# Brendonovich/spacedrive

Measured on AMD Instinct MI355X. Metric: cas_id files/sec + full-file BLAKE3 GB/s + dedup rows/sec at 1/2/4/8 MI355X, higher is better.
Workload: dtype u32; 1 GPU; identifier job step: config2 (1M files/GPU) cas_id + cas_id->Object grouping + Object write set (one fused pass on one GPU; at N > 1 hash-sharded over RCCL, each owner writing its share of the write set, padded exchange); parallelism=dp1 (files) + hash-sharded dedup, RCCL all-to-all

## Files before the change

### spacedrive_amd/csrc/b3_batch.hip

```cpp
#include <errno.h>
#include <stdlib.h>

#include <algorithm>
#include <atomic>

#include "b3_device.hpp"
#include "internal.hpp"
#include "scan_device.hpp"

namespace sdgpu {

namespace {

constexpr int kThreads = 256;

__device__ __forceinline__ void load_cv(const uint32_t* p, uint32_t cv[8]) {
  const uint4 a = reinterpret_cast<const uint4*>(p)[0];
  const uint4 b = reinterpret_cast<const uint4*>(p)[1];
  cv[0] = a.x; cv[1] = a.y; cv[2] = a.z; cv[3] = a.w;
  cv[4] = b.x; cv[5] = b.y; cv[6] = b.z; cv[7] = b.w;
}

__device__ __forceinline__ void store_cv(uint32_t* p, const uint32_t cv[8]) {
  reinterpret_cast<uint4*>(p)[0] = make_uint4(cv[0], cv[1], cv[2], cv[3]);
// ... 52 lines not shown
  if (rem == 0) return 0u;
  const uint32_t rem_bytes = len - 4 * q * B3_CHUNK_LEN;
  const uint32_t rem_blocks = rem_bytes == 0 ? 1u : (rem_bytes + 63) / 64;
  return rem_blocks + (rem - 1);
}

__device__ __forceinline__ void bins3(uint32_t len, bool ok, uint32_t& b0, uint32_t& b1) {
  b0 = b1 = kBins;
  if (!ok) return;
  const uint32_t lw = leaf_work3(len);
  if (lw) b0 = parent_bin(lw);
  const uint32_t q = units_of(len);
  if (q) b1 = parent_bin(q + (n_chunks_of(len) > 4 * q ? 1u : 0u));
}

struct Range3 {
  uint32_t lo, hi;
};
__device__ __forceinline__ Range3 block_range3(uint32_t n) {
  const uint32_t per = (n + gridDim.x - 1) / gridDim.x;
  const uint32_t lo = min(n, blockIdx.x * per);
  return {lo, min(n, lo + per)};
}

__device__ __forceinline__ bool msg_ok(uint64_t o, uint32_t l, uint32_t max_len,
                                       uint64_t arena_bytes) {
  return l <= max_len && (o & 15u) == 0 && o <= arena_bytes && l <= arena_bytes - o;
}

template <uint32_t kSkip>
constexpr uint32_t kAlignOf = kSkip ? 8u : 16u;

template <uint32_t kSkip>
__device__ __forceinline__ bool pass_msg(uint64_t o, uint32_t l, const uint8_t* __restrict__ whole,
                                         uint32_t i, uint32_t max_len, uint64_t arena_bytes,
                                         uint32_t& hl) {
  static_assert(kSkip == 0 || kSkip == 8, "the cas message or its body");
  bool ok = msg_ok(o, l, max_len, arena_bytes);
  hl = l;
  if constexpr (kSkip != 0) {
    ok = ok && l >= kSkip && whole[i] != 0;
    hl = l - kSkip;
  }
  return ok;
}

template <uint32_t kSkip>
__device__ __forceinline__ bool over_capacity(const uint32_t* d_units, uint32_t n, uint64_t cap,
                                              const uint32_t* grab) {
  if constexpr (kSkip != 0) return grab[1] != 0;
  return static_cast<uint64_t>(*d_units) + n > cap;
}

template <uint32_t kSkip>
__global__ __launch_bounds__(kThreads) void k_plan3(const uint64_t* __restrict__ off,
                                                    const uint32_t* __restrict__ len, uint32_t n,
                                                    uint32_t max_len, uint64_t arena_bytes,
                                                    uint32_t* __restrict__ units,
                                                    uint32_t* __restrict__ hist,
                                                    uint32_t* __restrict__ grab,
                                                    int32_t* __restrict__ status,
                                                    uint32_t out_words, uint32_t* __restrict__ out,
                                                    const uint8_t* __restrict__ whole,
                                                    uint8_t* __restrict__ has,
                                                    const uint32_t* d_units, uint64_t cap) {
  __shared__ uint32_t h[2][kBins];
  for (uint32_t t = threadIdx.x; t < 2 * kBins; t += kThreads) (&h[0][0])[t] = 0;
  if (blockIdx.x == 0 && threadIdx.x == 0) {
    *grab = 0;
    if constexpr (kSkip != 0) grab[1] = over_capacity<0>(d_units, n, cap, nullptr) ? 1u : 0u;
  }
  __syncthreads();
  const Range3 r = block_range3(n);
  for (uint32_t i = r.lo + threadIdx.x; i < r.hi; i += kThreads) {
    uint32_t l;
    const bool ok = pass_msg<kSkip>(off[i], len[i], whole, i, max_len, arena_bytes, l);
    units[i] = ok ? units_of(l) : 0u;
    if (status) status[i] = ok ? 0 : -EINVAL;
    if constexpr (kSkip != 0) has[i] = ok ? 1 : 0;
    if (!ok)
      for (uint32_t w = 0; w < out_words; ++w) out[i * out_words + w] = 0u;
    uint32_t b0, b1;
    bins3(l, ok, b0, b1);
    if (b0 < kBins) atomicAdd(&h[0][b0], 1u);
    if (b1 < kBins) atomicAdd(&h[1][b1], 1u);
  }
  __syncthreads();
  for (uint32_t t = threadIdx.x; t < 2 * kBins; t += kThreads)
    hist[static_cast<size_t>(t) * gridDim.x + blockIdx.x] = (&h[0][0])[t];
}

template <uint32_t kSkip>
__global__ __launch_bounds__(kThreads) void k_scatter3(const uint64_t* __restrict__ off,
                                                       const uint32_t* __restrict__ len, uint32_t n,
                                                       uint32_t max_len, uint64_t arena_bytes,
                                                       uint64_t cap, const uint32_t* __restrict__ d_units,
                                                       int32_t* __restrict__ status,
                                                       uint32_t out_words, uint32_t* __restrict__ out,
                                                       const uint32_t* __restrict__ unit_base,
                                                       const uint32_t* __restrict__ hist_scan,
                                                       uint32_t* __restrict__ order,
                                                       uint32_t* __restrict__ unit_msg,
                                                       const uint8_t* __restrict__ whole,
                                                       uint8_t* __restrict__ has,
                                                       const uint32_t* __restrict__ grab) {
  __shared__ uint32_t cur[2][kBins], cnt[2][kBins];
  const Range3 r = block_range3(n);
  if (over_capacity<kSkip>(d_units, n, cap, grab)) {
    for (uint32_t i = r.lo + threadIdx.x; i < r.hi; i += kThreads) {
      if (status) status[i] = -ENOBUFS;
      if constexpr (kSkip != 0) has[i] = 0;
      for (uint32_t w = 0; w < out_words; ++w) out[i * out_words + w] = 0u;
    }
    return;
  }
  for (uint32_t t = threadIdx.x; t < 2 * kBins; t += kThreads) {
    (&cur[0][0])[t] = hist_scan[static_cast<size_t>(t) * gridDim.x + blockIdx.x];
    (&cnt[0][0])[t] = 0;
  }
  __syncthreads();
  for (uint32_t i0 = r.lo; i0 < r.hi; i0 += kThreads) {
    const uint32_t i = i0 + threadIdx.x;
    uint32_t b0 = kBins, b1 = kBins, l0 = 0, l1 = 0;
    if (i < r.hi) {
      uint32_t l;
      const bool ok = pass_msg<kSkip>(off[i], len[i], whole, i, max_len, arena_bytes, l);
      bins3(l, ok, b0, b1);
      if (b0 < kBins) l0 = atomicAdd(&cnt[0][b0], 1u);
      if (b1 < kBins) l1 = atomicAdd(&cnt[1][b1], 1u);
      const uint32_t q = ok ? units_of(l) : 0u;
      const uint32_t ub = unit_base[i];
      for (uint32_t g = 0; g < q; ++g) unit_msg[ub + g] = i;
    }
    __syncthreads();
    if (b0 < kBins) order[cur[0][b0] + l0] = i;
    if (b1 < kBins) order[cur[1][b1] + l1] = i;
    __syncthreads();
    for (uint32_t t = threadIdx.x; t < 2 * kBins; t += kThreads) {
      (&cur[0][0])[t] += (&cnt[0][0])[t];
      (&cnt[0][0])[t] = 0;
    }
    __syncthreads();
  }
}

template <uint32_t kSkip>
__device__ __forceinline__ void unit_item(const uint8_t* __restrict__ arena,
                                          const uint64_t* __restrict__ off,
                                          const uint32_t* __restrict__ unit_msg,
                                          const uint32_t* __restrict__ unit_base, uint32_t u,
                                          uint32_t* __restrict__ cvs) {
  const uint32_t m = unit_msg[u];
  const uint32_t ub = unit_base[m];
  const uint32_t g = u - ub;
  const uint32_t j0 = 4 * g;
  const uint8_t* p = arena + off[m] + kSkip + static_cast<uint64_t>(j0) * B3_CHUNK_LEN;
  constexpr uint32_t kA = kAlignOf<kSkip>;
  uint32_t a[8], b[8], c[8];
  b3_chunk_full<kA>(p, j0, a);
  b3_chunk_full<kA>(p + 1024, j0 + 1, b);
  b3_parent(a, a, b, 0u);
  b3_chunk_full<kA>(p + 2048, j0 + 2, b);
  b3_chunk_full<kA>(p + 3072, j0 + 3, c);
  b3_parent(b, b, c, 0u);
  b3_parent(c, a, b, 0u);
  store_cv(cvs + static_cast<uint64_t>(ub + m + g) * 8, c);
}

template <uint32_t kAlign>
__device__ __forceinline__ void chunk_any(const uint8_t* __restrict__ p, uint32_t l, uint32_t j,
                                          uint32_t root_flag, uint32_t cv[8]) {
  const uint32_t clen = min(B3_CHUNK_LEN, l - j * B3_CHUNK_LEN);
  const uint8_t* cp = p + static_cast<uint64_t>(j) * B3_CHUNK_LEN;
  if (clen == B3_CHUNK_LEN && root_flag == 0)
    b3_chunk_full<kAlign>(cp, j, cv);
  else
    b3_chunk<kAlign>(cp, clen, j, root_flag, cv);
}

template <uint32_t kSkip>
__device__ __forceinline__ void msg_item(const uint8_t* __restrict__ arena,
                                         const uint64_t* __restrict__ off,
                                         const uint32_t* __restrict__ len,
                                         const uint32_t* __restrict__ unit_base, uint32_t m,
                                         uint32_t* __restrict__ cvs, uint32_t out_words,
                                         uint32_t* __restrict__ out) {
  const uint32_t l = len[m] - kSkip;
  const uint32_t nch = n_chunks_of(l), q = units_of(l);
  const uint32_t rem = nch - 4 * q;
  const uint8_t* p = arena + off[m] + kSkip;
  const uint32_t rootf = q == 0 ? B3_ROOT : 0u;
// ... 411 lines not shown
          break;
        }
        const uint64_t now = wall_clock64();
        if (now - t_last > idle_ticks || now - t_start > life_ticks) break;
        __builtin_amdgcn_s_sleep(2);
      }
      s_go = go;
    }
    __syncthreads();
    const uint32_t go = s_go;
    if (go == 0) break;
    const uint64_t t_seen = wall_clock64();
    const uint32_t l = min(s_len, kHostStageMax), out_words = min(s_words, 16u);
    stage_message(stage, msg, l);
    __syncthreads();
    const uint64_t t_loaded = wall_clock64();
    uint32_t h0 = 0, h1 = 0;
    quad_hash_staged(L, stage, l, cvr, h0, h1);
    if (t < 64) {
      uint32_t dg[8];
#pragma unroll
      for (int w = 0; w < 8; ++w) dg[w] = __shfl(w < 4 ? h0 : h1, w & 3);
      if (t == 0) {
        for (uint32_t w = 0; w < out_words; ++w)
          __hip_atomic_store(&mb->digest[w], w < 8 ? dg[w] : 0u, __ATOMIC_RELAXED,
                             __HIP_MEMORY_SCOPE_SYSTEM);
        __hip_atomic_store(&mb->t_seen, t_seen, __ATOMIC_RELAXED, __HIP_MEMORY_SCOPE_SYSTEM);
        __hip_atomic_store(&mb->t_loaded, t_loaded, __ATOMIC_RELAXED, __HIP_MEMORY_SCOPE_SYSTEM);
        __hip_atomic_store(&mb->t_done, wall_clock64(), __ATOMIC_RELAXED, __HIP_MEMORY_SCOPE_SYSTEM);
        __hip_atomic_store(&mb->done, go, __ATOMIC_RELEASE, __HIP_MEMORY_SCOPE_SYSTEM);
        last_seq = go;
      }
    }
    t_last = wall_clock64();
    __syncthreads();
  }
  if (t == 0) __hip_atomic_store(&mb->state, kSvcExited, __ATOMIC_RELEASE, __HIP_MEMORY_SCOPE_SYSTEM);
}

}

namespace {

template <uint32_t kSkip>
hipError_t batch_pass_launch(const uint8_t* arena, uint64_t arena_bytes, const uint64_t* off,
                             const uint32_t* len, const uint8_t* whole, uint32_t n,
                             uint32_t max_len, uint32_t out_words, uint8_t* out, uint8_t* has,
                             int32_t* status, const BatchWork& w, hipStream_t s, KTimer* timer) {
  if (n == 0) return hipSuccess;
  uint32_t* o = reinterpret_cast<uint32_t*>(out);
  const uint32_t nb = std::min<uint32_t>(kSortBlocks, (n + kThreads - 1) / kThreads);
  const uint32_t nh = 2 * kBins * nb;
  const uint64_t cap = w.max_chunks;
  k_plan3<kSkip><<<nb, kThreads, 0, s>>>(off, len, n, max_len, arena_bytes, w.n_chunks, w.hist,
                                         w.grab, status, out_words, o, whole, has, w.total, cap);
  scan::exclusive(w.n_chunks, n, w.chunk_base, w.block_sums, w.total, s);
  scan::exclusive(w.hist, nh, w.hist, w.hist_sums, nullptr, s);
  k_scatter3<kSkip><<<nb, kThreads, 0, s>>>(off, len, n, max_len, arena_bytes, cap, w.total, status,
                                            out_words, o, w.chunk_base, w.hist, w.order,
                                            w.chunk_msg, whole, has, w.grab);
  const uint32_t* d_r = w.hist + static_cast<size_t>(kBins) * nb;
  {
    KScope k(timer, kSkip ? "body_leaves" : "cas_leaves", s);
    k_leaves3<kSkip><<<leaves3_grid(), kThreads, 0, s>>>(arena, off, len, w.chunk_msg, w.chunk_base,
                                                         w.total, w.order, d_r, w.grab, w.cvs,
                                                         out_words, o, n, cap);
  }
  {
    KScope k(timer, kSkip ? "body_fold" : "cas_fold", s);
    k_fold3<kSkip><<<(n + kThreads - 1) / kThreads, kThreads, 0, s>>>(
        len, w.chunk_base, w.order, d_r, w.hist + nh, w.cvs, out_words, o, w.total, n, cap, w.grab);
  }
  return hipGetLastError();
}

}

hipError_t batch_hash_launch(const uint8_t* arena, uint64_t arena_bytes, const uint64_t* off,
                             const uint32_t* len, uint32_t n, uint32_t max_len,
                             uint32_t out_words, uint8_t* out, int32_t* status,
                             const BatchWork& w, hipStream_t s, KTimer* timer) {
  return batch_pass_launch<0>(arena, arena_bytes, off, len, nullptr, n, max_len, out_words, out,
                              nullptr, status, w, s, timer);
}

hipError_t batch_body_launch(const uint8_t* arena, uint64_t arena_bytes, const uint64_t* off,
                             const uint32_t* len, const uint8_t* whole, uint32_t n,
                             uint32_t max_len, uint8_t* out32, uint8_t* has, const BatchWork& w,
                             hipStream_t s, KTimer* timer) {
  return batch_pass_launch<8>(arena, arena_bytes, off, len, whole, n, max_len, 8, out32, has,
                              nullptr, w, s, timer);
}

}

namespace sdgpu {

size_t small_split_scratch_bytes() {
  return (kSplitMaxMsgs + static_cast<size_t>(kSplitMaxMsgs) * kSplitMaxGroups * 8) * 4;
}

hipError_t small_split_launch(const uint8_t* arena, const uint64_t* off, const uint32_t* len,
                              uint32_t n, uint32_t max_len, uint32_t max_chunks,
                              uint32_t out_words, uint8_t* out, int32_t* status, uint32_t* scratch,
                              hipStream_t s, KTimer* timer) {
  if (n == 0) return hipSuccess;
  if (n > kSplitMaxMsgs || max_chunks > kSmallMaxChunks || !scratch) return hipErrorInvalidValue;
  const uint32_t gmax = std::max<uint32_t>(1, (max_chunks + kSplitGroupChunks - 1) / kSplitGroupChunks);
  KScope k(timer, "cas_small_split", s);
  k_small_split<<<n * gmax, kSplitThreads, 0, s>>>(arena, off, len, max_len, gmax, out_words,
                                                   reinterpret_cast<uint32_t*>(out), status, scratch);
  return hipGetLastError();
}
// ... 51 lines not shown
```

### spacedrive_amd/csrc/bucket_part_device.hpp

```cpp
#pragma once

#include "part_device.hpp"

namespace sdgpu {
namespace {

constexpr uint32_t kMaxBucketBits = 15;

template <typename In, bool kInitRep>
__global__ __launch_bounds__(kPartThreads) void k_part_scatter_rec(
    In in, uint64_t n, uint32_t skip, uint32_t bits, const uint32_t* __restrict__ offs,
    uint4* __restrict__ rec, uint32_t* __restrict__ rep) {
  extern __shared__ __attribute__((aligned(16))) uint32_t cur[];
  const uint32_t nbins = 1u << bits;
  for (uint32_t b = threadIdx.x; b < nbins; b += kPartThreads)
    cur[b] = offs[static_cast<uint64_t>(b) * gridDim.x + part_block()];
  __syncthreads();
  uint64_t t0, t1;
  tile_of(n, gridDim.x, t0, t1);
  constexpr int U = kUnroll;
  for (uint64_t i0 = t0 + threadIdx.x; i0 < t1; i0 += U * kPartThreads) {
    RowBatch<U> q;
    in.template load_many<U>(i0, kPartThreads, t1, i0, q);
#pragma unroll
    for (int u = 0; u < U; ++u) {
      const uint64_t i = i0 + static_cast<uint64_t>(u) * kPartThreads;
      const uint32_t r = in.rank_of(q, u);
      if (kInitRep && q.in[u]) rep[i] = r;
      if (!in.valid_of(q, u)) continue;
      const uint64_t h = in_hash<In>(in.key_of(q, u));
      const uint32_t p = atomicAdd(&cur[digit_of(h, skip, bits)], 1u);
      rec[p] = make_uint4(static_cast<uint32_t>(h), static_cast<uint32_t>(h >> 32), r,
                          in.row_of(q, u));
    }
  }
}

constexpr uint32_t kRunMaxBins = 64;
template <typename In, bool kInitRep, bool kRec12 = false>
__global__ __launch_bounds__(kPartThreads) void k_part_scatter_runs(
    In in, uint64_t n, uint32_t skip, uint32_t bits, const uint32_t* __restrict__ offs,
    uint4* __restrict__ rec, uint32_t* __restrict__ rep, uint32_t fbits,
    uint32_t* __restrict__ fine, uint32_t* __restrict__ ovf) {
  constexpr int U = 4;
  constexpr uint32_t R = U * kPartThreads;
  using RecT = typename std::conditional<kRec12, uint3, uint4>::type;
  __shared__ RecT buf[R];
  RecT* __restrict__ out = reinterpret_cast<RecT*>(rec);
  __shared__ uint32_t cnt[kRunMaxBins], base[kRunMaxBins + 1], cur[kRunMaxBins];
  __shared__ uint32_t fc[1u << (kMaxBucketBits - 1)];
  const uint32_t nbins = 1u << bits, nfine = 1u << fbits;
  if (threadIdx.x < nbins)
    cur[threadIdx.x] = offs[static_cast<uint64_t>(threadIdx.x) * gridDim.x + part_block()];
  for (uint32_t b = threadIdx.x; b < nfine / 2; b += kPartThreads) fc[b] = 0;
  bool over = false;
  uint64_t t0, t1;
  tile_of(n, gridDim.x, t0, t1);
  auto round = [&](const RowBatch<U>& q, uint64_t i0) {
    if (threadIdx.x < nbins) cnt[threadIdx.x] = 0;
    lds_barrier();
    uint32_t dg[U], lr[U];
    RecT rq[U];
#pragma unroll
    for (int u = 0; u < U; ++u) {
      const uint64_t i = i0 + threadIdx.x + static_cast<uint64_t>(u) * kPartThreads;
      dg[u] = ~0u;
      if (!q.in[u]) continue;
      const uint32_t r = in.rank_of(q, u);
      if (kInitRep) rep[i] = r;
// ... 750 lines not shown
```

### spacedrive_amd/csrc/dedup.hip

```cpp
#include <cerrno>
#include <cstdlib>

#include "bucket_part_device.hpp"
#include "group_device.hpp"
#include "scan_device.hpp"

namespace sdgpu {
namespace {

constexpr uint64_t kBucketRows = 3072;
uint32_t bucket_bits_for(uint64_t n) {
  uint32_t bits = 1;
  while (bits < kMaxBucketBits && (n >> bits) > kBucketRows) ++bits;
  return bits;
}

enum class Path { kDirect, kStaged12, kTwoLevelRuns, kTwoLevelHist };
static_assert(kMaxBucketBits - kStage2Bits <= 6, "coarse digits fit k_part_scatter_runs");
static_assert(kStage2Blocks <= kPartBlocks && kPartBlocks % kStage2Blocks == 0,
              "second-pass blocks per segment");
constexpr uint32_t kStage2Coarse = kPartBlocks / kStage2Blocks;
static_assert((sizeof(uint32_t) << kStageBits) <= (64u << 10), "no hipFuncSetAttribute needed");

struct ForcedPlan {
// ... 105 lines not shown
bool rank_in_z(const In& in) {
  if constexpr (std::is_same<In, RowsIn>::value) return !in.rank;
  else return std::is_same<In, RecRankIn>::value;
}
template <typename In>
uint32_t z_rank_base(const In& in) {
  if constexpr (std::is_same<In, RowsIn>::value) return in.rank_base;
  else return 0u;
}

template <typename In, typename Out>
struct GroupCall {
  In in;
  uint64_t n;
  uint32_t chunk_rows;
  uint32_t* rep;
  bool init_rep;
  Out out;
  GroupLayout L;
  hipStream_t s;
  KTimer* timer;
};

template <typename F>
void with_flag(bool b, F f) {
  b ? f(std::true_type{}) : f(std::false_type{});
}
template <typename In, typename F>
void with_sink(const KeylessSink& xs, F f) {
  if constexpr (std::is_same<In, RowsIn>::value) {
    if (xs.st) return f(std::true_type{});
  }
  f(std::false_type{});
}

template <typename In, typename Out>
void hist_launch(const GroupCall<In, Out>& c, uint32_t bits, uint32_t* hist,
                 uint32_t* zero = nullptr, bool blk_major = false) {
  const KeylessSink xs = sink_of(c.out);
  const size_t lds = sizeof(uint32_t) << bits;
  with_sink<In>(xs, [&](auto sunk) {
    constexpr bool kX = decltype(sunk)::value;
    k_part_hist<In, kX><<<kPartBlocks, kPartThreads, lds, c.s>>>(
        c.in, c.n, kShardBits, bits, 0, hist, zero, blk_major, kX ? xs : KeylessSink{});
  });
}

template <bool kRec12, typename In, typename Out>
hipError_t group_kernel_launch(const GroupCall<In, Out>& c) {
  const uint32_t nb = 1u << c.L.bits;
  const ChunkOf chunk_of = ChunkOf::make(c.chunk_rows);
  KScope k(c.timer, "bucket_group", c.s);
  if (c.L.path == Path::kDirect)
    k_bucket_group<Out><<<nb, kGroupThreads, 0, c.s>>>(c.L.rec, c.L.hist, kPartBlocks, chunk_of,
                                                       c.L.gkey, c.L.gmin, c.out);
  else if constexpr (kRec12)
    k_bucket_group12_pk<Out><<<nb, kGroupThreads, 0, c.s>>>(
        reinterpret_cast<const uint3*>(c.L.rec), z_rank_base(c.in), c.L.fbase, c.L.bits, chunk_of,
        c.L.gkey, c.L.gmin, c.out);
  else
    k_bucket_group_pk<Out><<<nb, kGroupThreads, 0, c.s>>>(c.L.rec, c.L.fbase, 1, c.L.bits, chunk_of,
                                                          c.L.gkey, c.L.gmin, c.out);
  return out_finish(c.out, nb, c.s);
}

template <typename In, typename Out>
hipError_t direct_launch(const GroupCall<In, Out>& c) {
  const GroupLayout& L = c.L;
  const uint32_t bits = L.bits, nb = 1u << bits;
  const size_t lds = sizeof(uint32_t) << bits;
  {
    KScope k(c.timer, "bucket_hist", c.s);
    hist_launch(c, bits, L.hist);
  }
  scan::exclusive(L.hist, static_cast<uint64_t>(nb) * kPartBlocks, L.hist, L.tiles, nullptr, c.s);
  {
    KScope k(c.timer, "bucket_scatter", c.s);
    with_flag(c.init_rep, [&](auto init) {
      constexpr bool kInit = decltype(init)::value;
      k_part_scatter_rec<In, kInit><<<kPartBlocks, kPartThreads, lds, c.s>>>(
          c.in, c.n, kShardBits, bits, L.hist, L.rec, c.rep);
    });
  }
  return group_kernel_launch<false>(c);
}

template <bool kRec12, typename In, typename Out>
hipError_t staged12_launch(const GroupCall<In, Out>& c) {
  const GroupLayout& L = c.L;
  constexpr uint32_t nb = 1u << kStageBits;
  {
    KScope k(c.timer, "bucket_hist", c.s);
    hist_launch(c, kStageBits, L.fine, nullptr, true);
    k_fine_scan<kPartBlocks, 1><<<nb / 64, 1024, 0, c.s>>>(L.fine, nb, L.fE, L.ftot, L.ovf);
  }
  {
    KScope k(c.timer, "bucket_scatter", c.s);
    with_flag(c.init_rep, [&](auto init) {
      constexpr bool kInit = decltype(init)::value;
      if constexpr (!kRec12)
        k_part_scatter_rec_staged<In, kInit><<<kPartBlocks, kPartThreads, 0, c.s>>>(
            c.in, c.n, kShardBits, L.fE, L.rec, c.rep, nullptr, 0, L.ftot, L.fbase);
      else if constexpr (!kInit || std::is_same<In, RowsIn>::value)
        k_part_scatter_ws<In, kInit><<<kPartBlocks, kPartThreads, 0, c.s>>>(
            c.in, c.n, kShardBits, L.fE, L.ftot, reinterpret_cast<uint3*>(L.rec), c.rep, L.fbase);
    });
  }
  return group_kernel_launch<kRec12>(c);
}

template <bool kRec12, typename In, typename Out>
hipError_t two_level_runs_launch(const GroupCall<In, Out>& c) {
  using RecT = typename std::conditional<kRec12, uint3, uint4>::type;
  const GroupLayout& L = c.L;
  const uint32_t nfine = 1u << L.bits, nseg = 1u << L.cbits, skip2 = kShardBits + L.cbits;
  k_zero_runs<<<1, 64, 0, c.s>>>(L.segtot, L.ovf);
  {
    KScope k(c.timer, "bucket_scatter1", c.s);
    const KeylessSink xs = sink_of(c.out);
    auto coarse = [&](auto init, auto sunk) {
      constexpr bool kX = decltype(sunk)::value;
      k_part_private<In, decltype(init)::value, kRec12, kX><<<kPartBlocks, kPartThreads, 0, c.s>>>(
          c.in, c.n, kShardBits, L.cbits, L.rec1, c.rep, L.bits, L.fine, L.ovf, L.run_s, L.run_l,
          L.rounds, L.segtot, kX ? xs : KeylessSink{});
    };
    with_sink<In>(xs, [&](auto sunk) {
      if constexpr (decltype(sunk)::value)
        coarse(std::false_type{}, sunk);
      else
        with_flag(c.init_rep, [&](auto init) { coarse(init, sunk); });
    });
  }
  {
    KScope k(c.timer, "bucket_fine_scan", c.s);
// ... 138 lines not shown
```

### spacedrive_amd/csrc/group_device.hpp

```cpp
#pragma once

#include "part_device.hpp"

namespace sdgpu {
namespace {

constexpr int kGroupThreads = 1024;
constexpr uint32_t kLdsSlots = 6144;
constexpr uint32_t kLdsCap = 4608;
constexpr uint64_t kEmpty = ~0ull;
constexpr uint32_t kPadRow = 0xFFFFFFFFu;

__device__ __forceinline__ uint32_t lds_slot(uint64_t h) {
  return static_cast<uint32_t>((static_cast<uint64_t>(static_cast<uint32_t>(h)) * kLdsSlots) >> 32);
}

__device__ __forceinline__ uint32_t lds_step(uint64_t h) {
  return 1u + 6u * (static_cast<uint32_t>(h) & 1023u);
}

__device__ __forceinline__ uint32_t next_slot(uint32_t h, uint32_t step) {
  const uint32_t s = h + step;
  return s >= kLdsSlots ? s - kLdsSlots : s;
}

__device__ __forceinline__ uint64_t global_slot(uint64_t h, uint64_t tsize) {
  return h & (tsize - 1);
}

constexpr int kPer = (kLdsCap + kGroupThreads - 1) / kGroupThreads;

struct RepOut {
  static constexpr int kScratch = 1;
  uint32_t* rep;
  template <int kSteps>
  __device__ __forceinline__ void emit(const bool (&)[kSteps], const bool (&lk)[kSteps],
                                       const uint32_t (&)[kSteps], const uint32_t (&w)[kSteps],
                                       const uint32_t (&f)[kSteps], uint32_t, uint32_t,
                                       uint32_t*) const {
#pragma unroll
    for (int j = 0; j < kSteps; ++j)
      if (lk[j]) rep[w[j]] = f[j];
  }
};
__device__ __forceinline__ uint32_t block_sum(uint32_t v, uint32_t* sw) {
#pragma unroll
  for (int d = 32; d > 0; d >>= 1) v += __shfl_xor(v, d);
  if (__lane_id() == 0) sw[threadIdx.x >> 6] = v;
  __syncthreads();
  uint32_t t = 0;
  for (uint32_t w = 0; w < blockDim.x / 64; ++w) t += sw[w];
  __syncthreads();
  return t;
}
__global__ __launch_bounds__(1024) void k_list_finish(const uint32_t* __restrict__ lcnt,
// ... 336 lines not shown
  __syncthreads();
  bool lk[kP];
  uint32_t r[kP], w[kP], f[kP];
#pragma unroll
  for (int j = 0; j < kP; ++j) {
    r[j] = q[j].z;
    w[j] = q[j].w;
    f[j] = lmin[own1[j] - 1u];
    lk[j] = live[j] && r[j] != f[j] && chunk_of(r[j]) != chunk_of(f[j]);
  }
  out.template emit<kP>(live, lk, r, w, f, start, end, scr);
}

template <int kP, typename Src, typename Out>
__device__ __forceinline__ void group_packed_load(Src rec, uint32_t start, uint32_t end,
                                                  uint32_t bits, ChunkOf chunk_of, const Out& out,
                                                  uint64_t* tab, uint32_t* lmin, uint32_t* scr) {
  uint4 q[kP];
#pragma unroll
  for (int j = 0; j < kP; ++j) q[j] = rec(min(start + threadIdx.x + j * kGroupThreads, end - 1));
#pragma unroll
  for (int j = 0; j < kP; ++j)
    if (start + threadIdx.x + j * kGroupThreads >= end) q[j].w = kPadRow;
  group_packed_regs(q, start, end, bits, chunk_of, out, tab, lmin, scr);
}

template <typename Src, typename Out>
__device__ __forceinline__ void group_bucket_packed(Src rec, uint32_t start, uint32_t end,
                                                    uint32_t bits, ChunkOf chunk_of,
                                                    uint64_t* __restrict__ gkey,
                                                    uint32_t* __restrict__ gmin, const Out& out,
                                                    uint64_t* tab, uint32_t* lmin,
                                                    uint32_t& special_min, uint32_t* scr) {
  const uint32_t m = end - start;
  if (m == 0) {
    out_init(out, scr);
    out_done(out, end, scr);
    return;
  }
  if (m > kPkCap) {
    group_bucket_global(rec, start, end, chunk_of, gkey, gmin, out, special_min, scr);
    return;
  }
  static_assert(kPkCap <= 4 * kGroupThreads, "four records per thread hold a bucket");
  if (m <= 3 * kGroupThreads)
    group_packed_load<3>(rec, start, end, bits, chunk_of, out, tab, lmin, scr);
  else
    group_packed_load<4>(rec, start, end, bits, chunk_of, out, tab, lmin, scr);
  out_done(out, end, scr);
}

template <typename Out>
__global__ __launch_bounds__(kGroupThreads, 8) void k_bucket_group(
    const uint4* __restrict__ rec, const uint32_t* __restrict__ offs, uint32_t P,
    ChunkOf chunk_of, uint64_t* __restrict__ gkey, uint32_t* __restrict__ gmin, Out out) {
  __shared__ uint64_t lkey[kLdsSlots];
  __shared__ uint32_t lmin[kLdsSlots];
  __shared__ uint32_t special_min;
  __shared__ uint32_t scr[Out::kScratch];
  const uint32_t b = blockIdx.x;
  const uint32_t start = offs[static_cast<uint64_t>(b) * P];
  const uint32_t end = offs[static_cast<uint64_t>(b + 1) * P];
  uint4 q_reg[kPer];
  load_bucket(Rec16Src{rec}, start, end, q_reg);
  group_bucket(Rec16Src{rec}, start, end, q_reg, chunk_of, gkey, gmin, out, lkey, lmin,
               special_min, scr);
}

template <typename Out>
__global__ __launch_bounds__(kGroupThreads, 8) void k_bucket_group_pk(
    const uint4* __restrict__ rec, const uint32_t* __restrict__ offs, uint32_t P, uint32_t bits,
    ChunkOf chunk_of, uint64_t* __restrict__ gkey, uint32_t* __restrict__ gmin, Out out) {
  __shared__ uint64_t tab[kPkSlots];
  __shared__ uint32_t lw[kPkWords];
  static_assert(Out::kScratch <= 2, "scratch fits the word area");
  uint32_t* lmin = lw;
  uint32_t& special_min = lw[kPkCap];
  uint32_t* scr = lw + kPkCap + 1;
  const uint32_t b = blockIdx.x;
  group_bucket_packed(Rec16Src{rec}, offs[static_cast<uint64_t>(b) * P],
                      offs[static_cast<uint64_t>(b + 1) * P], bits, chunk_of, gkey, gmin, out, tab,
                      lmin, special_min, scr);
}

template <typename Out>
__global__ __launch_bounds__(kGroupThreads, 8) void k_bucket_group12_pk(
    const uint3* __restrict__ rec, uint32_t rank_base, const uint32_t* __restrict__ offs,
    uint32_t bits, ChunkOf chunk_of, uint64_t* __restrict__ gkey, uint32_t* __restrict__ gmin,
    Out out) {
  __shared__ uint64_t tab[kPkSlots];
  __shared__ uint32_t lw[kPkWords];
  static_assert(Out::kScratch <= 2, "scratch fits the word area");
  uint32_t* lmin = lw;
  uint32_t& special_min = lw[kPkCap];
  uint32_t* scr = lw + kPkCap + 1;
  const uint32_t b = blockIdx.x;
  group_bucket_packed(Rec12Src{rec, rank_base}, offs[b], offs[b + 1], bits, chunk_of, gkey, gmin,
                      out, tab, lmin, special_min, scr);
}

}
}
```

### spacedrive_amd/csrc/scan_device.hpp

```cpp
#pragma once

#include <hip/hip_runtime.h>
#include <stdint.h>

namespace sdgpu {
namespace scan {

constexpr int kThreads = 256;
constexpr uint32_t kTile = 1024;

inline uint32_t tiles_for(uint64_t n) { return static_cast<uint32_t>((n + kTile - 1) / kTile); }

__global__ __launch_bounds__(kThreads) static void k_tiles(const uint32_t* __restrict__ in,
                                                           uint64_t n, uint32_t* __restrict__ out,
                                                           uint32_t* __restrict__ tile_sums) {
  __shared__ uint32_t wsum[kThreads / 64];
  const uint64_t base = static_cast<uint64_t>(blockIdx.x) * kTile + threadIdx.x * 4;
  const uint32_t lane = threadIdx.x & 63u, w = threadIdx.x >> 6;
  uint32_t v[4];
  uint32_t s = 0;
#pragma unroll
  for (int k = 0; k < 4; ++k) {
    v[k] = base + k < n ? in[base + k] : 0u;
    s += v[k];
// ... 27 lines not shown
                                                             uint32_t ntiles,
                                                             uint32_t* __restrict__ out_total_slot,
                                                             uint32_t* __restrict__ total) {
  __shared__ uint32_t wsum[kSumThreads / 64];
  const uint32_t lane = threadIdx.x & 63u, w = threadIdx.x >> 6;
  uint32_t carry = 0;
  for (uint32_t b0 = 0; b0 < ntiles; b0 += kSumThreads) {
    const uint32_t i = b0 + threadIdx.x;
    const uint32_t v = i < ntiles ? tile_sums[i] : 0u;
    uint32_t inc = v;
#pragma unroll
    for (int d = 1; d < 64; d <<= 1) {
      const uint32_t o = __shfl_up(inc, d);
      if (lane >= static_cast<uint32_t>(d)) inc += o;
    }
    if (lane == 63) wsum[w] = inc;
    __syncthreads();
    uint32_t pre = 0, blk = 0;
    for (uint32_t k = 0; k < kSumThreads / 64; ++k) {
      const uint32_t x = wsum[k];
      pre += k < w ? x : 0u;
      blk += x;
    }
    if (i < ntiles) tile_sums[i] = carry + pre + inc - v;
    carry += blk;
    __syncthreads();
  }
  if (threadIdx.x == 0) {
    if (out_total_slot) *out_total_slot = carry;
    if (total) *total = carry;
  }
}

__global__ __launch_bounds__(kThreads) static void k_add(uint32_t* __restrict__ out, uint64_t n,
                                                         const uint32_t* __restrict__ tile_sums) {
  const uint64_t i = static_cast<uint64_t>(blockIdx.x) * kThreads + threadIdx.x;
  if (i < n) out[i] += tile_sums[i / kTile];
}

inline void exclusive(const uint32_t* in, uint64_t n, uint32_t* out, uint32_t* tile_sums,
                      uint32_t* total, hipStream_t s) {
  const uint32_t tiles = tiles_for(n);
  if (tiles == 0) {
    (void)hipMemsetAsync(out, 0, sizeof(uint32_t), s);
    if (total) (void)hipMemsetAsync(total, 0, sizeof(uint32_t), s);
    return;
  }
  k_tiles<<<tiles, kThreads, 0, s>>>(in, n, out, tile_sums);
  k_sums<<<1, kSumThreads, 0, s>>>(tile_sums, tiles, out + n, total);
  k_add<<<static_cast<uint32_t>((n + kThreads - 1) / kThreads), kThreads, 0, s>>>(out, n,
                                                                                   tile_sums);
}

}
}
```

### spacedrive_amd/csrc/shard.cpp

```cpp
#include <fcntl.h>
#include <stdlib.h>
#include <string.h>
#include <sys/mman.h>
#include <sys/stat.h>
#include <unistd.h>

#include <atomic>
#include <chrono>
#include <string>
#include <memory>
#include <thread>
#include <vector>

#include <rccl/rccl.h>

#include "ctx.hpp"

using namespace sdgpu;

namespace {

struct RankJob {
  sdgpu_ctx* c = nullptr;
  sdgpu_comm* comm = nullptr;
// ... 1271 lines not shown
                              uint32_t* d_count, void* stream) {
  if (!x || !d_count || (cap && (!d_key || !d_value))) return -EINVAL;
  std::lock_guard<std::mutex> g(x->ctx->mu);
  SD_TRY(hipSetDevice(x->ctx->device));
  hipStream_t s = pick(x->ctx, stream);
  SD_TRY(index_export_launch(x->ref, d_key, d_value, cap, d_count, s, x->ctx->kt()));
  return 0;
}

int sdgpu_index_add_objects_device(sdgpu_index* x, const uint64_t* d_key, const uint32_t* d_handle,
                                   uint64_t n, uint32_t world, uint32_t rank, void* stream) {
  if (!x || (n && (!d_key || !d_handle)) || world == 0 || world > 64 || rank >= world)
    return -EINVAL;
  std::lock_guard<std::mutex> g(x->ctx->mu);
  SD_TRY(hipSetDevice(x->ctx->device));
  hipStream_t s = pick(x->ctx, stream);
  SD_TRY_RC(index_reserve(x, n, s));
  SD_TRY(index_objects_launch(x->ref, d_key, d_handle, n, world, rank, s));
  return 0;
}

int sdgpu_group_rows_indexed_device(sdgpu_ctx* c, sdgpu_index* x, const uint64_t* d_key,
                                    const uint8_t* d_has_key, const uint32_t* d_rank, uint64_t n,
                                    uint32_t chunk_rows, uint32_t* d_rep, void* stream) {
  if (!c || !x || x->ctx->device != c->device || chunk_rows == 0 ||
      (n && (!d_key || !d_rep)))
    return -EINVAL;
  if (n >= (1ull << 32)) return -EINVAL;
  if (!d_rank && n > kRepExisting) return -EINVAL;
  std::lock_guard<std::mutex> g(c->mu);
  SD_TRY(hipSetDevice(c->device));
  hipStream_t s = pick(c, stream);
  if (n == 0) return 0;
  SD_TRY_RC(ensure_dev(c, c->xs_recv, n + 256));
  GroupInput in;
  in.key = d_key;
  in.valid = d_has_key;
  in.rank = d_rank;
  in.n = n;
  return group_with_index(c, x, in, chunk_rows, d_rep, static_cast<uint8_t*>(c->xs_recv.p), s);
}

int sdgpu_group_link_device(sdgpu_ctx* c, sdgpu_index* x, const uint64_t* d_key,
                            const uint8_t* d_has_key, const uint8_t* d_valid,
                            const uint32_t* d_rank, uint32_t first_rank, uint64_t n,
                            uint32_t chunk_rows, uint32_t* d_who, uint32_t* d_obj,
                            uint32_t* d_counts, void* stream) {
  if (!c || chunk_rows == 0 || !d_counts || (n && (!d_key || !d_who || !d_obj))) return -EINVAL;
  if (x && x->ctx->device != c->device) return -EINVAL;
  if (n >= (1ull << 31) || (!d_rank && first_rank + n > (1ull << 31))) return -EINVAL;
  std::lock_guard<std::mutex> g(c->mu);
  SD_TRY(hipSetDevice(c->device));
  hipStream_t s = pick(c, stream);
  SD_TRY(hipMemsetAsync(d_counts, 0, 3 * sizeof(uint32_t), s));
  if (n == 0) return 0;
  SD_TRY_RC(ensure_dev(c, c->dedup_ws, dedup_workspace_bytes(n, !x && d_has_key)));
  SD_TRY_RC(ensure_dev(c, c->link_ws, extra_workspace_bytes(n)));
  GroupInput in;
  in.key = d_key;
  in.valid = d_has_key;
  in.rank = d_rank;
  in.rank_base = first_rank;
  in.n = n;
  if (!x) {
    SD_TRY(dedup_list_launch(in, chunk_rows, d_who, d_obj, d_counts, c->dedup_ws.p, s, c->kt(),
                             true, d_valid));
    return 0;
  }
  const size_t o_mask = align_up(4 * n, 256);
  SD_TRY_RC(ensure_dev(c, c->xs_recv, o_mask + n + 256));
  uint32_t* hitrep = static_cast<uint32_t*>(c->xs_recv.p);
  uint8_t* mask = static_cast<uint8_t*>(c->xs_recv.p) + o_mask;
  SD_TRY_RC(index_reserve(x, n, s));
  SD_TRY(index_probe_launch(x->ref, in, chunk_rows, hitrep, mask, s, c->kt()));
  GroupInput gi = in;
  gi.valid = mask;
  SD_TRY(dedup_list_launch(gi, chunk_rows, d_who, d_obj, d_counts, c->dedup_ws.p, s, c->kt()));
  SD_TRY(extra_list_launch(d_has_key, d_valid, mask, hitrep, d_rank, first_rank, n, d_who, d_obj,
                           d_counts, c->link_ws.p, s, c->kt()));
  SD_TRY(index_creators_launch(x->ref, in, hitrep, mask, s, c->kt()));
  return 0;
}

int sdgpu_dedup_batch(sdgpu_ctx* c, sdgpu_index* x, const uint64_t* key, const uint8_t* has_key,
                      uint32_t first_rank, uint32_t n, uint32_t chunk_rows, uint32_t* rep) {
  if (!c || chunk_rows == 0 || (n && (!key || !has_key || !rep))) return -EINVAL;
  if (n == 0) return 0;
  if (static_cast<uint64_t>(first_rank) + n > kRepExisting) return -EINVAL;
  {
    std::lock_guard<std::mutex> g(c->mu);
    SD_TRY(hipSetDevice(c->device));
  }
  const size_t o_has = align_up(8ull * n, 256), o_rank = align_up(o_has + n, 256),
               o_rep = align_up(o_rank + 4ull * n, 256), total = align_up(o_rep + 4ull * n, 256);
  uint8_t* d = nullptr;
  if (hipMalloc(&d, total) != hipSuccess) return -ENOMEM;
  if (sdgpu::poison_ws() && sdgpu::poison_dev(d, total, "dedup_batch_rows") != 0) {
    (void)hipFree(d);
    return -EIO;
  }
  std::vector<uint32_t> rank(n);
  for (uint32_t i = 0; i < n; ++i) rank[i] = first_rank + i;
  hipStream_t s = c->stream;
  int rc = 0;
  do {
    if (hipMemcpyAsync(d, key, 8ull * n, hipMemcpyHostToDevice, s) != hipSuccess ||
        hipMemcpyAsync(d + o_has, has_key, n, hipMemcpyHostToDevice, s) != hipSuccess ||
// ... 214 lines not shown
```

Measured before the change: 75.60 million files/s.

## Replace three-kernel exclusive scans with single-pass ticketed tiled scan, defer tile add

Replaces the tiles/sums/add three-kernel exclusive scan with one kernel that scans tiles locally, and the last block (chosen by an atomic ticket) scans the tile sums. The final per-element tile-sum add is dropped, and consumers (scatter, bucket group) add the tile offset on read. The two scans in the batch path are fused into one launch. Plan/scatter kernels move to 1024 threads, and a redundant memset is skipped in the dedup path. This cuts kernel launches and full passes over the scanned arrays, but it relies on ticket reset and on the workspace having a spare slot after the tile sums for the ticket.

After: 75.88 million files/s (median of 6 runs). No clear change (+0.4%).

```diff
diff --git a/spacedrive_amd/csrc/b3_batch.hip b/spacedrive_amd/csrc/b3_batch.hip
--- a/spacedrive_amd/csrc/b3_batch.hip
+++ b/spacedrive_amd/csrc/b3_batch.hip
@@ -128,8 +128,10 @@
   return static_cast<uint64_t>(*d_units) + n > cap;
 }
 
-template <uint32_t kSkip>
-__global__ __launch_bounds__(kThreads) void k_plan3(const uint64_t* __restrict__ off,
+constexpr int kPlanThreads = 1024;
+
+template <uint32_t kSkip>
+__global__ __launch_bounds__(kPlanThreads) void k_plan3(const uint64_t* __restrict__ off,
                                                     const uint32_t* __restrict__ len, uint32_t n,
                                                     uint32_t max_len, uint64_t arena_bytes,
                                                     uint32_t* __restrict__ units,
@@ -139,16 +141,20 @@
                                                     uint32_t out_words, uint32_t* __restrict__ out,
                                                     const uint8_t* __restrict__ whole,
                                                     uint8_t* __restrict__ has,
-                                                    const uint32_t* d_units, uint64_t cap) {
+                                                    const uint32_t* d_units, uint64_t cap,
+                                                    uint32_t* __restrict__ ticket_u,
+                                                    uint32_t* __restrict__ ticket_h) {
   __shared__ uint32_t h[2][kBins];
-  for (uint32_t t = threadIdx.x; t < 2 * kBins; t += kThreads) (&h[0][0])[t] = 0;
+  for (uint32_t t = threadIdx.x; t < 2 * kBins; t += kPlanThreads) (&h[0][0])[t] = 0;
   if (blockIdx.x == 0 && threadIdx.x == 0) {
     *grab = 0;
+    *ticket_u = 0;
+    *ticket_h = 0;
     if constexpr (kSkip != 0) grab[1] = over_capacity<0>(d_units, n, cap, nullptr) ? 1u : 0u;
   }
   __syncthreads();
   const Range3 r = block_range3(n);
-  for (uint32_t i = r.lo + threadIdx.x; i < r.hi; i += kThreads) {
+  for (uint32_t i = r.lo + threadIdx.x; i < r.hi; i += kPlanThreads) {
     uint32_t l;
     const bool ok = pass_msg<kSkip>(off[i], len[i], whole, i, max_len, arena_bytes, l);
     units[i] = ok ? units_of(l) : 0u;
@@ -162,19 +168,21 @@
     if (b1 < kBins) atomicAdd(&h[1][b1], 1u);
   }
   __syncthreads();
-  for (uint32_t t = threadIdx.x; t < 2 * kBins; t += kThreads)
+  for (uint32_t t = threadIdx.x; t < 2 * kBins; t += kPlanThreads)
     hist[static_cast<size_t>(t) * gridDim.x + blockIdx.x] = (&h[0][0])[t];
 }
 
 template <uint32_t kSkip>
-__global__ __launch_bounds__(kThreads) void k_scatter3(const uint64_t* __restrict__ off,
+__global__ __launch_bounds__(kPlanThreads) void k_scatter3(const uint64_t* __restrict__ off,
                                                        const uint32_t* __restrict__ len, uint32_t n,
                                                        uint32_t max_len, uint64_t arena_bytes,
                                                        uint64_t cap, const uint32_t* __restrict__ d_units,
                                                        int32_t* __restrict__ status,
                                                        uint32_t out_words, uint32_t* __restrict__ out,
-                                                       const uint32_t* __restrict__ unit_base,
-                                                       const uint32_t* __restrict__ hist_scan,
+                                                       uint32_t* __restrict__ unit_base,
+                                                       const uint32_t* __restrict__ unit_tiles,
+                                                       uint32_t* __restrict__ hist_scan,
+                                                       const uint32_t* __restrict__ hist_tiles,
                                                        uint32_t* __restrict__ order,
                                                        uint32_t* __restrict__ unit_msg,
                                                        const uint8_t* __restrict__ whole,
@@ -183,19 +191,22 @@
   __shared__ uint32_t cur[2][kBins], cnt[2][kBins];
   const Range3 r = block_range3(n);
   if (over_capacity<kSkip>(d_units, n, cap, grab)) {
-    for (uint32_t i = r.lo + threadIdx.x; i < r.hi; i += kThreads) {
+    for (uint32_t i = r.lo + threadIdx.x; i < r.hi; i += kPlanThreads) {
       if (status) status[i] = -ENOBUFS;
       if constexpr (kSkip != 0) has[i] = 0;
       for (uint32_t w = 0; w < out_words; ++w) out[i * out_words + w] = 0u;
     }
     return;
   }
-  for (uint32_t t = threadIdx.x; t < 2 * kBins; t += kThreads) {
-    (&cur[0][0])[t] = hist_scan[static_cast<size_t>(t) * gridDim.x + blockIdx.x];
+  for (uint32_t t = threadIdx.x; t < 2 * kBins; t += kPlanThreads) {
+    const size_t h = static_cast<size_t>(t) * gridDim.x + blockIdx.x;
+    const uint32_t v = hist_scan[h] + hist_tiles[h / scan::kTile];
+    (&cur[0][0])[t] = v;
     (&cnt[0][0])[t] = 0;
+    if (t == kBins && blockIdx.x == 0) hist_scan[h] = v;
   }
   __syncthreads();
-  for (uint32_t i0 = r.lo; i0 < r.hi; i0 += kThreads) {
+  for (uint32_t i0 = r.lo; i0 < r.hi; i0 += kPlanThreads) {
     const uint32_t i = i0 + threadIdx.x;
     uint32_t b0 = kBins, b1 = kBins, l0 = 0, l1 = 0;
     if (i < r.hi) {
@@ -205,14 +216,15 @@
       if (b0 < kBins) l0 = atomicAdd(&cnt[0][b0], 1u);
       if (b1 < kBins) l1 = atomicAdd(&cnt[1][b1], 1u);
       const uint32_t q = ok ? units_of(l) : 0u;
-      const uint32_t ub = unit_base[i];
+      const uint32_t ub = unit_base[i] + unit_tiles[i / scan::kTile];
+      unit_base[i] = ub;
       for (uint32_t g = 0; g < q; ++g) unit_msg[ub + g] = i;
     }
     __syncthreads();
     if (b0 < kBins) order[cur[0][b0] + l0] = i;
     if (b1 < kBins) order[cur[1][b1] + l1] = i;
     __syncthreads();
-    for (uint32_t t = threadIdx.x; t < 2 * kBins; t += kThreads) {
+    for (uint32_t t = threadIdx.x; t < 2 * kBins; t += kPlanThreads) {
       (&cur[0][0])[t] += (&cnt[0][0])[t];
       (&cnt[0][0])[t] = 0;
     }
@@ -730,13 +742,15 @@
   const uint32_t nb = std::min<uint32_t>(kSortBlocks, (n + kThreads - 1) / kThreads);
   const uint32_t nh = 2 * kBins * nb;
   const uint64_t cap = w.max_chunks;
-  k_plan3<kSkip><<<nb, kThreads, 0, s>>>(off, len, n, max_len, arena_bytes, w.n_chunks, w.hist,
-                                         w.grab, status, out_words, o, whole, has, w.total, cap);
-  scan::exclusive(w.n_chunks, n, w.chunk_base, w.block_sums, w.total, s);
-  scan::exclusive(w.hist, nh, w.hist, w.hist_sums, nullptr, s);
-  k_scatter3<kSkip><<<nb, kThreads, 0, s>>>(off, len, n, max_len, arena_bytes, cap, w.total, status,
-                                            out_words, o, w.chunk_base, w.hist, w.order,
-                                            w.chunk_msg, whole, has, w.grab);
+  k_plan3<kSkip><<<nb, kPlanThreads, 0, s>>>(off, len, n, max_len, arena_bytes, w.n_chunks, w.hist,
+                                         w.grab, status, out_words, o, whole, has, w.total, cap,
+                                         scan::ticket_of(w.block_sums, n),
+                                         scan::ticket_of(w.hist_sums, nh));
+  scan::tiled(scan::tiled_of(w.n_chunks, n, w.chunk_base, w.block_sums, w.total),
+              scan::tiled_of(w.hist, nh, w.hist, w.hist_sums, nullptr), s);
+  k_scatter3<kSkip><<<nb, kPlanThreads, 0, s>>>(off, len, n, max_len, arena_bytes, cap, w.total, status,
+                                            out_words, o, w.chunk_base, w.block_sums, w.hist,
+                                            w.hist_sums, w.order, w.chunk_msg, whole, has, w.grab);
   const uint32_t* d_r = w.hist + static_cast<size_t>(kBins) * nb;
   {
     KScope k(timer, kSkip ? "body_leaves" : "cas_leaves", s);
diff --git a/spacedrive_amd/csrc/bucket_part_device.hpp b/spacedrive_amd/csrc/bucket_part_device.hpp
--- a/spacedrive_amd/csrc/bucket_part_device.hpp
+++ b/spacedrive_amd/csrc/bucket_part_device.hpp
@@ -1,6 +1,7 @@
 #pragma once
 
 #include "part_device.hpp"
+#include "scan_device.hpp"
 
 namespace sdgpu {
 namespace {
@@ -10,11 +11,12 @@
 template <typename In, bool kInitRep>
 __global__ __launch_bounds__(kPartThreads) void k_part_scatter_rec(
     In in, uint64_t n, uint32_t skip, uint32_t bits, const uint32_t* __restrict__ offs,
-    uint4* __restrict__ rec, uint32_t* __restrict__ rep) {
+    const uint32_t* __restrict__ tiles, uint4* __restrict__ rec, uint32_t* __restrict__ rep) {
   extern __shared__ __attribute__((aligned(16))) uint32_t cur[];
   const uint32_t nbins = 1u << bits;
+  const uint64_t nh = static_cast<uint64_t>(nbins) * gridDim.x;
   for (uint32_t b = threadIdx.x; b < nbins; b += kPartThreads)
-    cur[b] = offs[static_cast<uint64_t>(b) * gridDim.x + part_block()];
+    cur[b] = scan::at(offs, tiles, static_cast<uint64_t>(b) * gridDim.x + part_block(), nh);
   __syncthreads();
   uint64_t t0, t1;
   tile_of(n, gridDim.x, t0, t1);
diff --git a/spacedrive_amd/csrc/dedup.hip b/spacedrive_amd/csrc/dedup.hip
--- a/spacedrive_amd/csrc/dedup.hip
+++ b/spacedrive_amd/csrc/dedup.hip
@@ -181,8 +181,8 @@
   const ChunkOf chunk_of = ChunkOf::make(c.chunk_rows);
   KScope k(c.timer, "bucket_group", c.s);
   if (c.L.path == Path::kDirect)
-    k_bucket_group<Out><<<nb, kGroupThreads, 0, c.s>>>(c.L.rec, c.L.hist, kPartBlocks, chunk_of,
-                                                       c.L.gkey, c.L.gmin, c.out);
+    k_bucket_group<Out><<<nb, kGroupThreads, 0, c.s>>>(c.L.rec, c.L.hist, c.L.tiles, kPartBlocks,
+                                                       chunk_of, c.L.gkey, c.L.gmin, c.out);
   else if constexpr (kRec12)
     k_bucket_group12_pk<Out><<<nb, kGroupThreads, 0, c.s>>>(
         reinterpret_cast<const uint3*>(c.L.rec), z_rank_base(c.in), c.L.fbase, c.L.bits, chunk_of,
@@ -198,17 +198,18 @@
   const GroupLayout& L = c.L;
   const uint32_t bits = L.bits, nb = 1u << bits;
   const size_t lds = sizeof(uint32_t) << bits;
+  const uint64_t nh = static_cast<uint64_t>(nb) * kPartBlocks;
   {
     KScope k(c.timer, "bucket_hist", c.s);
-    hist_launch(c, bits, L.hist);
-  }
-  scan::exclusive(L.hist, static_cast<uint64_t>(nb) * kPartBlocks, L.hist, L.tiles, nullptr, c.s);
+    hist_launch(c, bits, L.hist, scan::ticket_of(L.tiles, nh));
+  }
+  scan::tiled(scan::tiled_of(L.hist, nh, L.hist, L.tiles, nullptr), c.s);
   {
     KScope k(c.timer, "bucket_scatter", c.s);
     with_flag(c.init_rep, [&](auto init) {
       constexpr bool kInit = decltype(init)::value;
       k_part_scatter_rec<In, kInit><<<kPartBlocks, kPartThreads, lds, c.s>>>(
-          c.in, c.n, kShardBits, bits, L.hist, L.rec, c.rep);
+          c.in, c.n, kShardBits, bits, L.hist, L.tiles, L.rec, c.rep);
     });
   }
   return group_kernel_launch<false>(c);
diff --git a/spacedrive_amd/csrc/group_device.hpp b/spacedrive_amd/csrc/group_device.hpp
--- a/spacedrive_amd/csrc/group_device.hpp
+++ b/spacedrive_amd/csrc/group_device.hpp
@@ -1,6 +1,7 @@
 #pragma once
 
 #include "part_device.hpp"
+#include "scan_device.hpp"
 
 namespace sdgpu {
 namespace {
@@ -443,15 +444,17 @@
 
 template <typename Out>
 __global__ __launch_bounds__(kGroupThreads, 8) void k_bucket_group(
-    const uint4* __restrict__ rec, const uint32_t* __restrict__ offs, uint32_t P,
-    ChunkOf chunk_of, uint64_t* __restrict__ gkey, uint32_t* __restrict__ gmin, Out out) {
+    const uint4* __restrict__ rec, const uint32_t* __restrict__ offs,
+    const uint32_t* __restrict__ tiles, uint32_t P, ChunkOf chunk_of, uint64_t* __restrict__ gkey,
+    uint32_t* __restrict__ gmin, Out out) {
   __shared__ uint64_t lkey[kLdsSlots];
   __shared__ uint32_t lmin[kLdsSlots];
   __shared__ uint32_t special_min;
   __shared__ uint32_t scr[Out::kScratch];
   const uint32_t b = blockIdx.x;
-  const uint32_t start = offs[static_cast<uint64_t>(b) * P];
-  const uint32_t end = offs[static_cast<uint64_t>(b + 1) * P];
+  const uint64_t nh = static_cast<uint64_t>(gridDim.x) * P;
+  const uint32_t start = scan::at(offs, tiles, static_cast<uint64_t>(b) * P, nh);
+  const uint32_t end = scan::at(offs, tiles, static_cast<uint64_t>(b + 1) * P, nh);
   uint4 q_reg[kPer];
   load_bucket(Rec16Src{rec}, start, end, q_reg);
   group_bucket(Rec16Src{rec}, start, end, q_reg, chunk_of, gkey, gmin, out, lkey, lmin,
diff --git a/spacedrive_amd/csrc/scan_device.hpp b/spacedrive_amd/csrc/scan_device.hpp
--- a/spacedrive_amd/csrc/scan_device.hpp
+++ b/spacedrive_amd/csrc/scan_device.hpp
@@ -103,5 +103,141 @@
                                                                                    tile_sums);
 }
 
-}
-}
+constexpr uint32_t kPer = 4;
+
+struct Tiled {
+  const uint32_t* in;
+  uint64_t n;
+  uint32_t* out;
+  uint32_t* tile_sums;
+  uint32_t* total;
+  uint32_t tiles;
+  uint32_t blocks;
+};
+
+inline Tiled tiled_of(const uint32_t* in, uint64_t n, uint32_t* out, uint32_t* tile_sums,
+                      uint32_t* total) {
+  const uint32_t tiles = tiles_for(n);
+  return Tiled{in, n, out, tile_sums, total, tiles, (tiles + kPer - 1) / kPer};
+}
+inline uint32_t* ticket_of(uint32_t* tile_sums, uint64_t n) { return tile_sums + tiles_for(n); }
+
+__device__ __forceinline__ uint32_t at(const uint32_t* __restrict__ out,
+                                       const uint32_t* __restrict__ tile_sums, uint64_t i,
+                                       uint64_t n) {
+  return out[i] + (i < n ? tile_sums[i / kTile] : 0u);
+}
+
+__global__ __launch_bounds__(kThreads) static void k_tiled(Tiled a, Tiled b) {
+  __shared__ uint32_t wsum[kPer][kThreads / 64];
+  __shared__ uint32_t s_last;
+  const bool second = blockIdx.x >= a.blocks;
+  const Tiled j = second ? b : a;
+  const uint32_t tile0 = (second ? blockIdx.x - a.blocks : blockIdx.x) * kPer;
+  const uint32_t lane = threadIdx.x & 63u, w = threadIdx.x >> 6;
+  uint32_t v[kPer][4], s[kPer], inc[kPer];
+#pragma unroll
+  for (uint32_t t = 0; t < kPer; ++t) {
+    const uint64_t base = static_cast<uint64_t>(tile0 + t) * kTile + threadIdx.x * 4;
+    if (base + 4 <= j.n) {
+      const uint4 q = *reinterpret_cast<const uint4*>(j.in + base);
+      v[t][0] = q.x, v[t][1] = q.y, v[t][2] = q.z, v[t][3] = q.w;
+    } else {
+#pragma unroll
+      for (int k = 0; k < 4; ++k) v[t][k] = base + k < j.n ? j.in[base + k] : 0u;
+    }
+    s[t] = inc[t] = v[t][0] + v[t][1] + v[t][2] + v[t][3];
+  }
+#pragma unroll
+  for (int d = 1; d < 64; d <<= 1) {
+#pragma unroll
+    for (uint32_t t = 0; t < kPer; ++t) {
+      const uint32_t o = __shfl_up(inc[t], d);
+      if (lane >= static_cast<uint32_t>(d)) inc[t] += o;
+    }
+  }
+  if (lane == 63) {
+#pragma unroll
+    for (uint32_t t = 0; t < kPer; ++t) wsum[t][w] = inc[t];
+  }
+  __syncthreads();
+  uint32_t tot[kPer];
+#pragma unroll
+  for (uint32_t t = 0; t < kPer; ++t) {
+    uint32_t pre = 0;
+    tot[t] = 0;
+#pragma unroll
+    for (int k = 0; k < kThreads / 64; ++k) {
+      const uint32_t x = wsum[t][k];
+      pre += static_cast<uint32_t>(k) < w ? x : 0u;
+      tot[t] += x;
+    }
+    const uint64_t base = static_cast<uint64_t>(tile0 + t) * kTile + threadIdx.x * 4;
+    uint32_t run = pre + inc[t] - s[t];
+    if (base + 4 <= j.n) {
+      uint4 q;
+      q.x = run, q.y = q.x + v[t][0], q.z = q.y + v[t][1], q.w = q.z + v[t][2];
+      *reinterpret_cast<uint4*>(j.out + base) = q;
+    } else {
+#pragma unroll
+      for (int k = 0; k < 4; ++k) {
+        if (base + k < j.n) j.out[base + k] = run;
+        run += v[t][k];
+      }
+    }
+  }
+  uint32_t* ticket = j.tile_sums + j.tiles;
+  if (threadIdx.x == 0) {
+#pragma unroll
+    for (uint32_t t = 0; t < kPer; ++t)
+      if (tile0 + t < j.tiles)
+        __hip_atomic_store(j.tile_sums + tile0 + t, tot[t], __ATOMIC_RELAXED,
+                           __HIP_MEMORY_SCOPE_AGENT);
+    const uint32_t drawn =
+        __hip_atomic_fetch_add(ticket, 1u, __ATOMIC_ACQ_REL, __HIP_MEMORY_SCOPE_AGENT);
+    s_last = drawn + 1 == j.blocks;
+  }
+  __syncthreads();
+  if (!s_last) return;
+  __builtin_amdgcn_fence(__ATOMIC_ACQUIRE, "agent");
+  uint32_t carry = 0;
+  for (uint32_t b0 = 0; b0 < j.tiles; b0 += kThreads) {
+    const uint32_t i = b0 + threadIdx.x;
+    const uint32_t x = i < j.tiles ? __hip_atomic_load(j.tile_sums + i, __ATOMIC_RELAXED,
+                                                       __HIP_MEMORY_SCOPE_AGENT)
+                                   : 0u;
+    uint32_t in2 = x;
+#pragma unroll
+    for (int d = 1; d < 64; d <<= 1) {
+      const uint32_t o = __shfl_up(in2, d);
+      if (lane >= static_cast<uint32_t>(d)) in2 += o;
+    }
+    if (lane == 63) wsum[0][w] = in2;
+    __syncthreads();
+    uint32_t p2 = 0, blk = 0;
+#pragma unroll
+    for (int k = 0; k < kThreads / 64; ++k) {
+      const uint32_t y = wsum[0][k];
+      p2 += static_cast<uint32_t>(k) < w ? y : 0u;
+      blk += y;
+    }
+    if (i < j.tiles) j.tile_sums[i] = carry + p2 + in2 - x;
+    carry += blk;
+    __syncthreads();
+  }
+  if (threadIdx.x == 0) {
+    j.out[j.n] = carry;
+    if (j.total) *j.total = carry;
+    __hip_atomic_store(ticket, 0u, __ATOMIC_RELAXED, __HIP_MEMORY_SCOPE_AGENT);
+  }
+}
+
+inline void tiled(const Tiled& a, hipStream_t s) {
+  k_tiled<<<a.blocks, kThreads, 0, s>>>(a, Tiled{nullptr, 0, nullptr, nullptr, nullptr, 0, 0});
+}
+inline void tiled(const Tiled& a, const Tiled& b, hipStream_t s) {
+  k_tiled<<<a.blocks + b.blocks, kThreads, 0, s>>>(a, b);
+}
+
+}
+}
diff --git a/spacedrive_amd/csrc/shard.cpp b/spacedrive_amd/csrc/shard.cpp
--- a/spacedrive_amd/csrc/shard.cpp
+++ b/spacedrive_amd/csrc/shard.cpp
@@ -1347,7 +1347,7 @@
   std::lock_guard<std::mutex> g(c->mu);
   SD_TRY(hipSetDevice(c->device));
   hipStream_t s = pick(c, stream);
-  SD_TRY(hipMemsetAsync(d_counts, 0, 3 * sizeof(uint32_t), s));
+  if (n == 0 || x) SD_TRY(hipMemsetAsync(d_counts, 0, 3 * sizeof(uint32_t), s));
   if (n == 0) return 0;
   SD_TRY_RC(ensure_dev(c, c->dedup_ws, dedup_workspace_bytes(n, !x && d_has_key)));
   SD_TRY_RC(ensure_dev(c, c->link_ws, extra_workspace_bytes(n)));
```
